# taconite/arah-release

Measured on AMD Instinct MI355X. Metric: rendered rays/sec, higher is better.
Workload: dtype f32 (operands as hi+lo f16 pairs on the f16 MFMA pipe, fp32 accumulate)

## Files before the change

arah_release_amd/csrc/arah_hip.hip:

```cpp
#include <hip/hip_runtime.h>
#include <stdint.h>
#include <stdlib.h>
#include <string.h>

#include <atomic>
#include <mutex>
#include <type_traits>

#include "../../include/arah_hip.h"
#include "pointwise.hpp"
#include "mlp.hpp"

using namespace arah;

namespace {

constexpr float kRootThresh = 1e-5f;
constexpr int kSphereIters = 50;
constexpr float kSurfaceRange = 0.05f;
constexpr float kClampDist = 0.1f;
constexpr int kBroydenSteps = 50;
constexpr float kDvg = 1.0f;
constexpr int kMaxVerts = 6912;
constexpr int kKnnThreads = 1024;
// ... 78 lines not shown
    d.vert_T = f.vert_T;
    d.bones = f.bones;
    d.scal = f.scalars;
    d.n_verts = f.n_verts;
    return d;
}

struct TierStatsRaw {
    unsigned long long rays, rays_surface, rays_promoted, rays_skipped, samples_p1, samples_p2, samples_skipped, witnesses;
    unsigned long long rays_untraced;
};
struct Counters {
    unsigned long long n_sdf_fwd, n_sdf_grad, n_skin_fwd, n_skin_jac, n_col, n_knn, n_density, n_canon, n_split_nonfinite;
    TierStatsRaw tier;
    unsigned long long n_canon_p2, n_density_p2;
    unsigned long long tier_snap[2];
    unsigned long long clk[8 * 16];
    unsigned long long clk_shade[8 * 16];
};
static_assert(offsetof(Counters, tier_snap) == sizeof(ArahCounters), "the head of Counters is the ABI's ArahCounters");
#ifdef ARAH_CLOCKS
typedef PhaseClk KernelClk;
#else
typedef NoClk KernelClk;
#endif

__device__ __forceinline__ void count_add(unsigned long long* c, int n) {
    if (c && n > 0) atomicAdd(c, (unsigned long long)n);
}

struct ColSegs {
    int n;
    int dst0[4], src0[4], len[4];
};

// ... 2401 lines not shown
        for (int s = 0; s < S; ++s)
            if (mask[base + s] != 0) step(s, z[base + s], shaded[base + s], nrm[base + s]);
    }
    step(S, 0.f, ps, pn);
    rgb[(size_t)i * 3] = any ? r : 0.f;
    rgb[(size_t)i * 3 + 1] = any ? g : 0.f;
    rgb[(size_t)i * 3 + 2] = any ? b : 0.f;
    if (acc) acc[i] = any ? fminf(fmaxf(wsum, 0.f), 1.f) : 0.f;
    vol_mask[i] = any ? 1 : 0;
    normal[(size_t)i * 3] = any ? nx : 0.f;
    normal[(size_t)i * 3 + 1] = any ? ny : 0.f;
    normal[(size_t)i * 3 + 2] = any ? nz : 0.f;
    depth[i] = any ? dz : 0.f;
}

__global__ void k_points_cam(FrameDev fr, int n, RaySet rs, const float* dists, const uint8_t* conv,
                             const float* points_hat_norm, const float* __restrict__ pose, float* points_cam) {
    const BodyConst bc = load_bc(fr);
    const int i = blockIdx.x * blockDim.x + threadIdx.x;
    if (i >= n) return;
    const V3 pw = ray_point(rs, i, dists[i]);
    const float wx = (pw.x - bc.trans[0]) + bc.trans[0], wy = (pw.y - bc.trans[1]) + bc.trans[1],
                wz = (pw.z - bc.trans[2]) + bc.trans[2];
    const float ax = fabsf(points_hat_norm[(size_t)i * 3]), ay = fabsf(points_hat_norm[(size_t)i * 3 + 1]),
                az = fabsf(points_hat_norm[(size_t)i * 3 + 2]);
    const bool surf = conv[i] && ax <= 1.0f && ay <= 1.0f && az <= 1.0f;
    for (int r = 0; r < 3; ++r) {
        const float v = pose[r * 4] * wx + pose[r * 4 + 1] * wy + pose[r * 4 + 2] * wz + pose[r * 4 + 3];
        points_cam[(size_t)i * 3 + r] = surf ? v : 0.f;
    }
// ... 38 lines not shown
    f32x4* spill;
    float *t, *far, *xcur, *Tcur, *x0raw, *grad_sdf, *jac_lbs;
    uint8_t* diverged;
    int* nn_idx;
    float *u_eval, *u_step, *u_gx, *u_Jinv, *err_best_ray, *xbest_ray, *zbest_ray;
    float *o_xnorm, *o_Tray, *o_start, *o_end, *o_acc;
    uint8_t* o_conv;
    float* q_err;
    float *o_z, *o_pts, *o_T;
    uint8_t* o_mask;
    uint8_t* q_smask;
    f32x4* shaded;
    int *listC, *listD;
    int* tcounts;
    uint8_t* ray_tier;
    size_t bytes;
};

Workspace carve(void* base, int n_rays, int n_steps) {
    Workspace w;
    Carver c{reinterpret_cast<char*>(base), 0};
    const size_t N = (size_t)(n_rays > 0 ? n_rays : 1), Q = N * (size_t)(n_steps > 0 ? n_steps : 1);
    w.ctr = c.take<Counters>(1);
    w.counts = c.take<int>(3 * kNumCounts);
    w.spill = c.take<f32x4>((size_t)kMaxGrid * kSpillPerWg);
    w.t = c.take<float>(N);
    w.far = c.take<float>(N);
    w.xcur = c.take<float>(N * 3);
    w.Tcur = c.take<float>(N * 16);
    w.x0raw = c.take<float>(N * 3);
// ... 15 lines not shown
    w.o_acc = c.take<float>(N);
    w.o_conv = c.take<uint8_t>(N);
    w.listA = c.take<int>(Q);
    w.listB = c.take<int>(Q);
    w.q_err = c.take<float>(Q);
    w.o_z = c.take<float>(Q);
    w.o_pts = c.take<float>(Q * 3);
    w.o_T = c.take<float>(Q * 16);
    w.o_mask = c.take<uint8_t>(Q);
    w.q_smask = c.take<uint8_t>(Q);
    w.shaded = c.take<f32x4>(Q);
    w.listC = c.take<int>(Q);
    w.listD = c.take<int>(Q);
    w.tcounts = c.take<int>(TC_COUNT);
    w.ray_tier = c.take<uint8_t>(N);
    w.bytes = align_up(c.off, 256);
    return w;
}

struct Knobs {
    int max_grid;
    int knn_group;
    int knn_below[3];
    int joint_bulk;
    int trace_bulk;
    int trace_small;
    bool train_b3;
    int canon_tier_wgs;
    int posed_canon;
};
// ... 812 lines not shown
    Workspace w = carve(const_cast<void*>(workspace), 1, 1);
    hipStream_t s = reinterpret_cast<hipStream_t>(stream);
    if (hipMemcpyAsync(h_out, w.ctr->clk, sizeof(w.ctr->clk) + sizeof(w.ctr->clk_shade), hipMemcpyDeviceToHost, s) != hipSuccess) return ARAH_E_LAUNCH;
    return hipStreamSynchronize(s) == hipSuccess ? ARAH_OK : ARAH_E_LAUNCH;
}
#endif

int arah_counters_read(const void* workspace, ArahCounters* h_out, void* stream) {
    if (!workspace || !h_out) return ARAH_E_BADARG;
    Workspace w = carve(const_cast<void*>(workspace), 1, 1);
    hipStream_t s = reinterpret_cast<hipStream_t>(stream);
    if (hipMemcpyAsync(h_out, w.ctr, sizeof(ArahCounters), hipMemcpyDeviceToHost, s) != hipSuccess) return ARAH_E_LAUNCH;
    return hipStreamSynchronize(s) == hipSuccess ? ARAH_OK : ARAH_E_LAUNCH;
}

int arah_sdf_eval(const ArahFrame* f, const float* x_norm, int32_t n, float* sdf, float* feat, float* grad,
                  void* workspace, size_t wbytes, void* stream) {
    if (!f || n < 0 || !workspace) return ARAH_E_BADARG;
    if (n == 0) return ARAH_OK;
    if (!x_norm || !sdf) return ARAH_E_BADARG;
    Workspace w = carve(workspace, 1, 1);
    if (wbytes < w.bytes) return ARAH_E_WORKSPACE;
    if (int arc = setup_attributes()) return arc;
    hipStream_t s = reinterpret_cast<hipStream_t>(stream);
    const FrameDev fd = to_dev(*f);
    const int g = grid_for(n, kTile);
    if (grad)
        LAUNCH_ENGINE(fd.split, (k_sdf_eval<true, true>), (k_sdf_eval<true, false>), dim3(g), dim3(kThreads), kLdsSdfGrad,
                      s, fd, x_norm, (const int*)nullptr, (const int*)nullptr, n, sdf, feat, grad, w.spill,
                      &w.ctr->n_sdf_fwd, &w.ctr->n_sdf_grad, 0);
// ... 1142 lines not shown
                         reinterpret_cast<hipStream_t>(stream));
    return check_launch();
}

static void launch_density(const FrameDev& fd, Workspace& w, const float* pts, long long Q, const int* list, const int* count,
                           int* next_list, int* next_count, hipStream_t s) {
    const int g = grid_for(Q, kTile);
    if (fd.split && Q >= 128ll * 1024)
        hipLaunchKernelGGL((k_density<true, 8>), dim3(min(num_cus(), grid_for(Q, 128))), dim3(kThreads), kLdsDensityWide, s, fd,
                           pts, list, count, w.shaded, next_list, next_count, &w.ctr->n_sdf_fwd, &w.ctr->n_density);
    else
        LAUNCH_ENGINE(fd.split, k_density<true>, k_density<false>, dim3(g), dim3(kThreads), kLdsSdfFwd, s, fd, pts, list, count,
                      w.shaded, next_list, next_count, &w.ctr->n_sdf_fwd, &w.ctr->n_density);
}

struct MapsOut {
    f32x4* nrm;
    float* normal;
    float* depth;
};

static int shade_tail(const ArahFrame* f, const ArahSampling* cfg, Workspace& w, const FrameDev& fd, const float* dirs,
                      const float* z, const float* pts, const float* T, const uint8_t* mask, int32_t n, const int* slist,
                      const int* scount, float* rgb, float* acc, uint8_t* vol_mask, const MapsOut* maps, hipStream_t s);

static int shade_impl(const ArahFrame* f, const ArahSampling* cfg, Workspace& w, const float* dirs, const float* z,
                      const float* pts, const float* T, const uint8_t* mask, int32_t n, float* rgb, float* acc,
                      uint8_t* vol_mask, const MapsOut* maps, hipStream_t s) {
    const int S = cfg->n_steps;
    const FrameDev fd = to_dev(*f);
    const long long Q = (long long)n * S;
    hipMemsetAsync(w.counts, 0, sizeof(int) * 3 * kNumCounts, s);
    hipLaunchKernelGGL(k_build_list, dim3((int)((Q + 4095) / 4096)), dim3(1024), 0, s, mask, (int)Q, w.listA, &w.counts[0]);
    const int g = grid_for(Q, kTile);
    const int* slist = w.listA;
    const int* scount = &w.counts[0];
    if (!cfg->full_shading) {
        if (cfg->ev_density[0] && cfg->ev_density[1]) hipEventRecord(reinterpret_cast<hipEvent_t>(cfg->ev_density[0]), s);
        launch_density(fd, w, pts, Q, (const int*)w.listA, (const int*)&w.counts[0], w.listB, &w.counts[1], s);
        if (cfg->ev_density[0] && cfg->ev_density[1]) hipEventRecord(reinterpret_cast<hipEvent_t>(cfg->ev_density[1]), s);
        slist = w.listB;
        scount = &w.counts[1];
    }
    return shade_tail(f, cfg, w, fd, dirs, z, pts, T, mask, n, slist, scount, rgb, acc, vol_mask, maps, s);
}

extern "C++" template <bool MAPS>
static void launch_shade(const ArahFrame* f, const ArahSampling* cfg, Workspace& w, const FrameDev& fd, const float* dirs,
                         const float* pts, const float* T, const int* slist, const int* scount, int g, f32x4* nrm,
                         hipStream_t s) {
    const int S = cfg->n_steps;
    const B3Nets b3 = b3_of(*f);
// ... 10 lines not shown
        LAUNCH_ENGINE(fd.split, (k_shade<true, true, false, MAPS>), (k_shade<true, false, false, MAPS>), dim3(g), dim3(kThreads),
                      lds_shade<true>(), s, fd, S, cfg->cano_view_dirs, dirs, pts, T, slist, scount, 0, w.shaded, w.spill,
                      &w.ctr->n_sdf_fwd, &w.ctr->n_sdf_grad, &w.ctr->n_col, b3, nrm);
    else
        LAUNCH_ENGINE(fd.split, (k_shade<false, true, false, MAPS>), (k_shade<false, false, false, MAPS>), dim3(g), dim3(kThreads),
                      lds_shade<false>(), s, fd, S, cfg->cano_view_dirs, dirs, pts, T, slist, scount, 0, w.shaded, w.spill,
                      &w.ctr->n_sdf_fwd, &w.ctr->n_sdf_grad, &w.ctr->n_col, b3, nrm);
}

static int shade_tail(const ArahFrame* f, const ArahSampling* cfg, Workspace& w, const FrameDev& fd, const float* dirs,
                      const float* z, const float* pts, const float* T, const uint8_t* mask, int32_t n, const int* slist,
                      const int* scount, float* rgb, float* acc, uint8_t* vol_mask, const MapsOut* maps, hipStream_t s) {
    const int S = cfg->n_steps;
    const long long Q = (long long)n * S;
    const int g = grid_for(Q, kTile);
    if (cfg->ev_shade[0] && cfg->ev_shade[1]) hipEventRecord(reinterpret_cast<hipEvent_t>(cfg->ev_shade[0]), s);
    if (maps) launch_shade<true>(f, cfg, w, fd, dirs, pts, T, slist, scount, g, maps->nrm, s);
    else launch_shade<false>(f, cfg, w, fd, dirs, pts, T, slist, scount, g, nullptr, s);
    if (cfg->ev_shade[0] && cfg->ev_shade[1]) hipEventRecord(reinterpret_cast<hipEvent_t>(cfg->ev_shade[1]), s);
    const bool chunk = S % 8 == 0 && (reinterpret_cast<uintptr_t>(z) & 15) == 0 && (reinterpret_cast<uintptr_t>(mask) & 7) == 0;
    const dim3 gc((n + 127) / 128), bc(128);
    if (maps) {
        if (chunk) hipLaunchKernelGGL(k_composite_maps<true>, gc, bc, 0, s, n, S, cfg->render_last_pt, z, mask, (const f32x4*)w.shaded,
                                      rgb, acc, vol_mask, (const f32x4*)maps->nrm, maps->normal, maps->depth);
        else hipLaunchKernelGGL(k_composite_maps<false>, gc, bc, 0, s, n, S, cfg->render_last_pt, z, mask, (const f32x4*)w.shaded,
                                rgb, acc, vol_mask, (const f32x4*)maps->nrm, maps->normal, maps->depth);
    } else if (chunk) hipLaunchKernelGGL(k_composite<true>, gc, bc, 0, s, n, S, cfg->render_last_pt, z, mask, (const f32x4*)w.shaded,
                                         rgb, acc, vol_mask);
    else hipLaunchKernelGGL(k_composite<false>, gc, bc, 0, s, n, S, cfg->render_last_pt, z, mask, (const f32x4*)w.shaded,
                            rgb, acc, vol_mask);
    return check_launch();
}

int arah_shade_points(const ArahFrame* f, const float* x_norm, const float* T, const float* dirs, int32_t n,
                      int32_t cano_view_dirs, int32_t shade_engine, float* rgbs, float* sdfn, void* workspace, size_t wbytes,
                      void* stream) {
// ... 1472 lines not shown
    Workspace w = carve(workspace, n, cfg->n_steps);
    if (wbytes < w.bytes) return ARAH_E_WORKSPACE;
    if (int arc = setup_attributes()) return arc;
    hipStream_t s = reinterpret_cast<hipStream_t>(stream);
    float* o_start = dists ? dists : w.o_start;
    uint8_t* o_conv = surface_conv ? surface_conv : w.o_conv;
    const uint8_t* skip = nullptr;
    if (cfg->occupancy) {
        OccBuf o = carve_occ(const_cast<void*>(cfg->occupancy));
        hipLaunchKernelGGL(k_tier_rays, dim3((n + 255) / 256), dim3(256), 0, s, n, make_rays(cam_loc, dirs, rays_per_cam), near_far,
                           (const OccInfo*)o.info, (const uint8_t*)o.dist, w.ray_tier, &w.ctr->tier);
        skip = w.ray_tier;
    }
    rc = trace_impl(f, w, cam_loc, rays_per_cam, dirs, near_far, n, 0, w.o_xnorm, w.o_Tray, o_conv, o_start, w.o_end, s, skip);
    if (rc) return rc;
    if (cfg->occupancy && !cfg->full_shading) {
        rc = render_tiers(f, cfg, w, cam_loc, rays_per_cam, dirs, near_far, o_conv, o_start, w.o_end, n, rgb,
                          acc ? acc : w.o_acc, vol_mask, maps, s);
        if (rc) return rc;
    } else {
        rc = sample_impl(f, cfg, w, cam_loc, rays_per_cam, dirs, near_far, o_conv, o_start, w.o_end, n, nullptr, nullptr,
                         nullptr, w.o_z, w.o_pts, w.o_T, w.o_mask, s);
        if (rc) return rc;
        rc = shade_impl(f, cfg, w, dirs, w.o_z, w.o_pts, w.o_T, w.o_mask, n, rgb, acc ? acc : w.o_acc, vol_mask, maps, s);
        if (rc) return rc;
    }
    if (points_cam)
        hipLaunchKernelGGL(k_points_cam, dim3((n + 255) / 256), dim3(256), 0, s, to_dev(*f), n,
                           make_rays(cam_loc, dirs, rays_per_cam), (const float*)o_start, (const uint8_t*)o_conv,
                           (const float*)w.o_xnorm, d_pose34, points_cam);
    return check_launch();
// ... 57 lines not shown
    const size_t off = align_up(c.off, 256);
    a.w = carve(base ? reinterpret_cast<char*>(base) + off : nullptr, n_rays, n_steps);
    a.bytes = off + a.w.bytes;
    return a;
}

extern "C" {
size_t arah_tier_audit_bytes(int32_t n_rays, int32_t n_steps) { return carve_audit(nullptr, n_rays, n_steps).bytes; }

int arah_tier_audit(const ArahFrame* f, const ArahSampling* cfg, const float* cam_loc, int32_t rays_per_cam, const float* dirs,
                    const float* near_far, int32_t n, int32_t rate_log2, uint32_t seed, void* audit_buf, size_t audit_bytes,
                    void* workspace, size_t wbytes, void* stream) {
    if (!f || !cfg || n < 0 || !workspace || !audit_buf) return ARAH_E_BADARG;
    int rc = check_sampling(cfg);
    if (rc) return rc;
    if (!cfg->occupancy || cfg->full_shading || rate_log2 < 0 || rate_log2 > 31) return ARAH_E_BADARG;
    if (n > 0 && (!cam_loc || !dirs || !near_far)) return ARAH_E_BADARG;
    const int S = cfg->n_steps;
    Workspace w = carve(workspace, n, S);
    if (wbytes < w.bytes) return ARAH_E_WORKSPACE;
    AuditBuf ab = carve_audit(audit_buf, n, S);
    if (audit_bytes < ab.bytes) return ARAH_E_WORKSPACE;
    if (int arc = setup_attributes()) return arc;
    hipStream_t s = reinterpret_cast<hipStream_t>(stream);
    Workspace& a = ab.w;
    hipMemsetAsync(a.ctr, 0, sizeof(Counters), s);
    hipLaunchKernelGGL(k_audit_begin, dim3(1), dim3(256), 0, s, ab.res, ab.aux, a.tcounts, (int)rate_log2, seed);
    if (n == 0) {
        hipLaunchKernelGGL(k_audit_finish, dim3(1), dim3(64), 0, s, ab.res, (const int*)ab.aux);
        return check_launch();
    }
// ... 169 lines not shown
```

arah_release_amd/hip.py:

```python
import ctypes as C
import os

import torch

_HERE = os.path.dirname(os.path.abspath(__file__))
LIB_PATH = os.environ.get("ARAH_LIB_PATH") or os.path.join(_HERE, "libarah_hip.so")

ARAH_MAX_STEPS = 128
COLOR_NO_VIEW_DIR = 0
COLOR_IDR = 1
PRECISION_SPLIT_F16 = 0
PRECISION_FP32 = 1


SHADE_ENGINE_DEFAULT, SHADE_ENGINE_FP32 = 0, 1
CANON_KERNEL_WAVE, CANON_KERNEL_TILE, CANON_KERNEL_WAVE_L2 = 0, 1, 2


def default_shade_engine():
    return SHADE_ENGINE_FP32 if os.environ.get("ARAH_SHADE_ENGINE", "b3") == "fp32" else SHADE_ENGINE_DEFAULT


def default_canon_kernel():
    return {"tile": CANON_KERNEL_TILE, "wave_l2": CANON_KERNEL_WAVE_L2}.get(os.environ.get("ARAH_CANON_KERNEL", "wave"), CANON_KERNEL_WAVE)
# ... 62 lines not shown
                ("d", _fp * 6)]


class ArahCounters(C.Structure):
    _fields_ = [("n_sdf_fwd", C.c_uint64), ("n_sdf_grad", C.c_uint64), ("n_skin_fwd", C.c_uint64),
                ("n_skin_jac", C.c_uint64), ("n_col", C.c_uint64), ("n_knn", C.c_uint64),
                ("n_density", C.c_uint64), ("n_canon", C.c_uint64), ("n_split_nonfinite", C.c_uint64),
                ("n_tier_rays", C.c_uint64), ("n_tier_rays_surface", C.c_uint64), ("n_tier_rays_promoted", C.c_uint64),
                ("n_tier_rays_skipped", C.c_uint64), ("n_tier_samples_p1", C.c_uint64), ("n_tier_samples_p2", C.c_uint64),
                ("n_tier_samples_skipped", C.c_uint64), ("n_tier_witnesses", C.c_uint64),
                ("n_tier_rays_untraced", C.c_uint64),
                ("n_canon_p2", C.c_uint64), ("n_density_p2", C.c_uint64)]


COUNTER_BYTES = C.sizeof(ArahCounters)


class ArahTierAudit(C.Structure):
    _fields_ = [("a_examined", C.c_uint64), ("a_violations", C.c_uint64), ("b_examined", C.c_uint64),
                ("b_converged", C.c_uint64), ("b_violations", C.c_uint64), ("c_examined", C.c_uint64),
                ("c_violations", C.c_uint64), ("n_first", C.c_uint64), ("first_index", C.c_int64 * 8),
                ("first_class", C.c_int32 * 8), ("min_ratio", C.c_float), ("rate_log2", C.c_int32), ("seed", C.c_uint32),
                ("reserved", C.c_int32)]


AUDIT_BYTES = C.sizeof(ArahTierAudit)

EXPORTS = ["arah_frame_bytes", "arah_prepare_frame", "arah_body_bytes", "arah_prepare_body", "arah_workspace_bytes", "arah_counters_reset",
           "arah_counters_read", "arah_sdf_eval", "arah_sdf_grid", "arah_rasterize", "arah_skin_lbs", "arah_skin_jacobian", "arah_color_eval",
           "arah_nearest_inverse_lbs", "arah_broyden3_lbs", "arah_joint_root_find", "arah_trace", "arah_sample_canonicalize",
           "arah_shade_composite", "arah_shade_points", "arah_render", "arah_shade_train_slab_bytes", "arah_shade_train_forward",
           "arah_shade_train_backward", "arah_composite_train_forward", "arah_composite_train_backward", "arah_gram_skinny_blocks", "arah_gram_skinny", "arah_colsum_blocks", "arah_colsum", "arah_inverse3x3", "arah_hsoftmax_train_forward", "arah_hsoftmax_train_backward", "arah_pose_tree_forward", "arah_pose_tree_backward", "arah_gemv_rows", "arah_mesh_query_scratch_bytes", "arah_mesh_query", "arah_dominant_kernel",
           "arah_skin_lbs_counted", "arah_marching_cubes_scratch_bytes", "arah_marching_cubes",
           "arah_marching_cubes_indexed_scratch_bytes", "arah_marching_cubes_indexed",
           "arah_occupancy_bytes", "arah_prepare_occupancy", "arah_occupancy_info", "arah_tier_debug", "arah_debug_samples",
           "arah_sample_depths_debug", "arah_cell_clusters_debug",
           "arah_sdf_grid_band_scratch_bytes", "arah_sdf_grid_band", "arah_tier_audit_bytes", "arah_tier_audit",
           "arah_tier_audit_debug", "arah_occupancy_clear_box", "arah_render_maps_bytes", "arah_render_maps",
           "arah_query_posed_bytes", "arah_query_posed", "arah_sdf_grid_posed_bytes", "arah_sdf_grid_posed",
           "arah_image_metrics_bytes", "arah_image_metrics",
           "arah_mesh_index_bytes", "arah_mesh_index_build", "arah_mesh_closest", "arah_surface_metrics_bytes", "arah_surface_metrics", "arah_face_area_cumsum",
           "arah_mesh_components_scratch_bytes", "arah_mesh_components", "arah_mesh_select_scratch_bytes", "arah_mesh_select",
           "arah_mesh_simplify_scratch_bytes", "arah_mesh_simplify",
           "arah_mesh_quadric_place_scratch_bytes", "arah_mesh_quadric_place",
# ... 235 lines not shown
            _check(load_library().arah_debug_samples(_ptr(self.buf), C.c_size_t(self.buf.numel()), C.c_int32(n_rays), C.c_int32(n_steps),
                                                     _ptr(out.get("z")), _ptr(out.get("pts")), _ptr(out.get("T")), _ptr(out.get("mask")),
                                                     _ptr(out.get("shaded")), _ptr(out.get("state")), _stream(d)), "arah_debug_samples")
        return out

    def ensure(self, n_rays, n_steps):
        need = load_library().arah_workspace_bytes(int(n_rays), int(n_steps))
        if self.buf is None or self.buf.numel() < need:
            old = self.buf
            with torch.cuda.device(self.device):
                self.buf = torch.empty(need, dtype=torch.uint8, device=self.device)
                if old is None:
                    _check(load_library().arah_counters_reset(_ptr(self.buf), _stream(self.device)),
                           "arah_counters_reset")
                else:
                    self.buf[:COUNTER_BYTES].copy_(old[:COUNTER_BYTES])
        return self.buf

    def reset_counters(self):
        with torch.cuda.device(self.device):
            _check(load_library().arah_counters_reset(_ptr(self.buf), _stream(self.device)), "arah_counters_reset")

    def counters(self):
        out = ArahCounters()
        with torch.cuda.device(self.device):
            _check(load_library().arah_counters_read(_ptr(self.buf), C.byref(out), _stream(self.device)),
                   "arah_counters_read")
        return {k: int(getattr(out, k)) for k, _ in ArahCounters._fields_}


OCC_NC, OCC_F, OCC_L, OCC_MAX_CELLS, OCC_MAX_VOX, OCC_ALIGN, TIER_BAND = 49, 3, 1.5, 12288, 1 << 22, 256, 18.0
OCC_MAX_FINE = OCC_MAX_CELLS * OCC_F ** 3
OCC_INFO_WORDS = 16
OCC_FIELDS = (("info", torch.int32, (OCC_INFO_WORDS,)), ("bits", torch.int32, (OCC_MAX_VOX // 32,)), ("dist", torch.uint8, (OCC_MAX_VOX,)),
              ("csdf", torch.float32, (OCC_NC ** 3,)), ("cpts", torch.float32, (OCC_NC ** 3, 3)),
              ("cell_lip", torch.float32, (OCC_MAX_CELLS,)), ("cell_stretch", torch.float32, (OCC_MAX_CELLS,)),
              ("fnorm", torch.float32, (OCC_MAX_FINE, 3)), ("fsdf", torch.float32, (OCC_MAX_FINE,)), ("iota", torch.int32, (OCC_MAX_FINE,)),
              ("sel_raw", torch.float32, (OCC_MAX_FINE, 3)), ("sel_bar", torch.float32, (OCC_MAX_FINE, 3)),
              ("sel_idx", torch.int32, (OCC_MAX_FINE,)), ("sel_of", torch.int32, (OCC_MAX_FINE,)))


def occupancy_layout():
    out, off = [], 0
# ... 115 lines not shown
        _same_device(*keep)
        nbytes = lib.arah_frame_bytes(C.byref(nets), C.byref(body))
        self.handle = ArahFrame()
        with _on_device(dev):
            self.buf = torch.empty(nbytes, dtype=torch.uint8, device=dev)
            _check(lib.arah_prepare_frame(C.byref(nets), C.byref(body), _ptr(self.buf), C.c_size_t(nbytes),
                                          C.byref(self.handle), _stream()), "arah_prepare_frame")
        self._keep = keep
        self.device = dev
        self.color_mode = int(color_mode)


class Sampling:

    def __init__(self, device, n_steps=64, n_near=16, n_far=16, cano_view_dirs=True, render_last_pt=False,
                 full_shading=False, shade_engine=None, canon_kernel=None):
        if n_steps < n_near + n_far + 1 or n_steps > ARAH_MAX_STEPS:
            raise ValueError("need n_near + n_far + 1 <= n_steps <= %d (ARAH_E_SAMPLING)" % ARAH_MAX_STEPS)
        self.lin_steps = torch.linspace(0.0, 1.0, n_steps, dtype=torch.float32).to(device)
        self.lin_near = torch.linspace(0.0, 1.0, n_near + 1, dtype=torch.float32).to(device)
        self.lin_far = torch.linspace(0.0, 1.0, max(n_far, 1), dtype=torch.float32).to(device)
        s = ArahSampling()
        s.n_steps, s.n_near, s.n_far = int(n_steps), int(n_near), int(n_far)
        s.cano_view_dirs, s.render_last_pt = int(bool(cano_view_dirs)), int(bool(render_last_pt))
        s.full_shading = int(bool(full_shading))
        s.lin_steps, s.lin_near, s.lin_far = _ptr(self.lin_steps), _ptr(self.lin_near), _ptr(self.lin_far)
        s.shade_engine = default_shade_engine() if shade_engine is None else int(shade_engine)
        s.canon_kernel = default_canon_kernel() if canon_kernel is None else int(canon_kernel)
        self.handle = s
        self._events = {}
        self.n_steps, self.n_near, self.n_far = n_steps, n_near, n_far

    def set_events(self, which, start=None, stop=None):
        field = getattr(self.handle, {"canon": "ev_canon", "density": "ev_density", "shade": "ev_shade", "canon2": "ev_canon2",
                                      "density2": "ev_density2"}[which])
        for ev in (start, stop):
            if ev is not None and not ev.cuda_event:
                ev.record()
        field[0] = start.cuda_event if start is not None else None
        field[1] = stop.cuda_event if stop is not None else None
# ... 1657 lines not shown
        raise ValueError("inverse3x3: (P, 3, 3) required")
    with _on_device(dev):
        out = torch.empty_like(mm)
        _check(lib.arah_inverse3x3(_ptr(mm), C.c_int32(mm.shape[0]), C.c_float(float(scale)), _ptr(out), _stream()),
               "arah_inverse3x3")
    return out


@_guarded
def render(frame, ws, sampling, cam_loc, dirs, near_far, pose34, tiered=False, maps=False):
    lib = load_library()
    cam, d, nf = _f32(cam_loc), _f32(dirs), _f32(near_far)
    n, S = d.shape[0], sampling.n_steps
    buf = ws.ensure(n, S)
    cfg = sampling.handle
    if tiered and not cfg.full_shading:
        occ = ws.occupancy(frame)
        buf = ws.buf
        cfg = ArahSampling.from_buffer_copy(sampling.handle)
        cfg.occupancy = occ.data_ptr()
    dev = d.device
    rgb = torch.empty(n, 3, device=dev)
    pcam = torch.empty(n, 3, device=dev)
    vol = torch.empty(n, dtype=torch.uint8, device=dev)
    acc = torch.empty(n, device=dev)
    dists = torch.empty(n, device=dev)
    conv = torch.empty(n, dtype=torch.uint8, device=dev)
    d_pose = _f32(pose34).reshape(-1)[:12].contiguous()
    if not maps:
        _check(lib.arah_render(C.byref(frame.handle), C.byref(cfg), _ptr(cam), C.c_int32(n // cam.shape[0]),
                               _ptr(d), _ptr(nf), _ptr(d_pose), C.c_int32(n), _ptr(rgb), _ptr(pcam), _ptr(vol), _ptr(acc),
# ... 40 lines not shown
```

arah_release_amd/renderer.py:

```python
import os

import numpy as np
import torch
import torch.nn as nn

from . import hip, training
from .nets import folded_weight


def draw_uniform(shape, device, tag):
    return torch.rand(shape, device=device)


def _emitted_sdf_layers(sdf_network):
    n = len(sdf_network)
    layers, freqs, phases = [], [], []
    for i in range(n - 1):
        lin = sdf_network[i][0]
        layers.append((lin.weights[0], lin.biases.reshape(-1)))
        freqs.append(lin.freq.reshape(-1))
        phases.append(lin.phase_shift.reshape(-1))
    last = sdf_network[n - 1]
    layers.append((last.weights[0], last.biases.reshape(-1)))
    return layers, torch.cat(freqs), torch.cat(phases)
# ... 196 lines not shown
                             "surface range, like every ARAH config")
        self.root_finding_threshold = root_finding_threshold
        self.sphere_tracing_iters = sphere_tracing_iters
        self.n_steps = n_steps
        self.near_surface_vol_samples = near_surface_vol_samples
        self.far_surface_vol_samples = far_surface_vol_samples
        self.surface_vol_range = surface_vol_range
        self.sample_bg_pts = sample_bg_pts
        self.low_vram = low_vram
        self.pending_bounds_ok = None
        self._ws = {}
        self._sampling = {}
        self.full_shading = os.environ.get("ARAH_FULL_SHADING", "0") == "1"
        self.shade_engine = None
        self.canon_kernel = None
        self._events = {}

    def workspace(self, device):
        device = torch.device(device)
        if device.type == "cuda" and device.index is None:
            device = torch.device("cuda", torch.cuda.current_device())
        key = (device, torch.cuda.current_stream(device).cuda_stream if device.type == "cuda" else 0)
        if key not in self._ws:
            if len(self._ws) >= 8:
                self._ws.pop(next(iter(self._ws)))
            self._ws[key] = hip.Workspace(device)
        return self._ws[key]

    def workspaces(self):
        return list(self._ws.values())

    def sampling(self, device, cano_view_dirs=True, render_last_pt=False, full_shading=None):
        full = bool(self.full_shading if full_shading is None else full_shading)
        key = (str(device), bool(cano_view_dirs), bool(render_last_pt), full, self.shade_engine, self.canon_kernel)
        if key not in self._sampling:
            sm = hip.Sampling(device, self.n_steps, self.near_surface_vol_samples, self.far_surface_vol_samples,
                              cano_view_dirs, render_last_pt, full, self.shade_engine, self.canon_kernel)
            for which, (a, b) in self._events.items():
                sm.set_events(which, a, b)
            self._sampling[key] = sm
        return self._sampling[key]

    def set_events(self, which, start=None, stop=None):
        if start is None or stop is None:
            self._events.pop(which, None)
        else:
            self._events[which] = (start, stop)
        for sm in self._sampling.values():
            sm.set_events(which, start, stop)

    def forward(self, sdf_network, skinning_model, cam_loc, ray_directions, body_bounds_intersections, loc,
                sc_factor, smpl_verts, smpl_verts_cano, skinning_weights, vol_feat, bone_transforms, trans,
# ... 162 lines not shown
               "surface_normals": None}
        if pred_weights is not None:
            out["pred_weights"] = pred_weights
        if inside_sdf is not None:
            out["inside_sdf"] = inside_sdf
        return out

    def _split_guard(self, ws, dev):
        key = (dev, id(ws))
        g = self._guard.get(key)
        if g is not None and self.guard_mode != "strict" and g["event"].query():
            ctr = g["host"].tolist()
            now = int(ctr[8])
            grew = now - g["seen"] if now >= g["seen"] else now
            g["seen"] = now
            d_col, d_den = ctr[4] - g["col"], ctr[6] - g["den"]
            g["col"], g["den"] = ctr[4], ctr[6]
            win_full, g["win_full"] = g["win_full"], False
            if d_den > 0 and d_col >= 0 and not win_full:
                self.shade_ratio = d_col / d_den
                self._shade_full = self.shade_ratio > 0.7
            tier_now = (ctr[13], ctr[14], ctr[15])
            d_t = [a - b for a, b in zip(tier_now, g["tier"])]
            g["tier"] = tier_now
            if min(d_t) >= 0 and sum(d_t) > 0:
                self.tier_share = d_t[2] / sum(d_t)
                self._tier_off = self.tier_share < 1.0 / 3.0
            if grew > 0:
                self.split_nonfinite += grew
                if self._precision != hip.PRECISION_FP32:
                    import warnings
                    warnings.warn("split-f16 engine: %d loop-C samples met activations outside the f16 range; following frames "
                                  "use the exact fp32 engine (ARAH_PRECISION=fp32)" % grew)
                    self._precision = hip.PRECISION_FP32
        if g is None:
            if len(self._guard) >= 8:
                self._guard.pop(next(iter(self._guard)))
            g = self._guard[key] = {"host": torch.zeros(hip.COUNTER_BYTES // 8, dtype=torch.int64).pin_memory(), "event": torch.cuda.Event(),
                                    "seen": 0, "col": 0, "den": 0, "win_full": False, "tier": (0, 0, 0)}
        return g

    def _split_guard_arm(self, g, ws, full=False):
        g["win_full"] = g["win_full"] or bool(full)
        g["host"].copy_(ws.buf[0:hip.COUNTER_BYTES].view(torch.int64), non_blocking=True)
        g["event"].record()

    def _tier_audit_mode(self):
        mode = self.tier_audit
        if mode not in ("off", "sample", "strict"):
            raise ValueError("tier_audit must be 'off', 'sample' or 'strict', not %r" % (mode,))
        return mode

    def _tier_audit_violated(self, res, where):
        import warnings
        self.tier_violations += res["violations"]
        self.tier_audit_last = res
        self.tiering = False
        warnings.warn("tiered forward: the audit of the sigma = +0 certificate found %d violation(s) (classes A/B/C: %d/%d/%d, "
                      "min sdf / beta %.3g); %s, and the following frames render untiered until `tiering` is set again"
# ... 653 lines not shown
```

include/arah_hip.h:

```cpp
#ifndef ARAH_HIP_H
#define ARAH_HIP_H

#include <stddef.h>
#include <stdint.h>

#ifdef __cplusplus
extern "C" {
#endif

#define ARAH_OK 0
#define ARAH_E_BADARG (-1)
#define ARAH_E_SHAPE (-2)
#define ARAH_E_WORKSPACE (-3)
#define ARAH_E_LAUNCH (-4)
#define ARAH_E_SAMPLING (-5)
#define ARAH_E_OVERFLOW (-6)

#define ARAH_MAX_STEPS 128
#define ARAH_N_JOINTS 24
#define ARAH_COLOR_NO_VIEW_DIR 0
#define ARAH_COLOR_IDR 1

#define ARAH_PRECISION_SPLIT_F16 0
#define ARAH_PRECISION_FP32 1
// ... 14 lines not shown
    int32_t precision;
} ArahNets;

typedef struct ArahBody {
    const float* verts;
    const float* vert_weights;
    const float* bones;
    const float* trans;
    const float* center;
    const float* coord_min;
    const float* coord_max;
    int32_t n_verts;
    const void* prepared;
} ArahBody;

enum { ARAH_SHADE_ENGINE_DEFAULT = 0 , ARAH_SHADE_ENGINE_FP32 = 1 };
enum { ARAH_CANON_KERNEL_WAVE = 0 , ARAH_CANON_KERNEL_TILE = 1,
       ARAH_CANON_KERNEL_WAVE_L2 = 2 };

typedef struct ArahSampling {
    int32_t n_steps, n_near, n_far;
    int32_t cano_view_dirs;
    int32_t render_last_pt;
    int32_t full_shading;
    const float* lin_steps;
    const float* lin_near;
    const float* lin_far;
    int32_t shade_engine;
    int32_t canon_kernel;
    void* ev_canon[2];
// ... 61 lines not shown
    uint64_t n_tier_rays, n_tier_rays_surface, n_tier_rays_promoted, n_tier_rays_skipped;
    uint64_t n_tier_samples_p1, n_tier_samples_p2, n_tier_samples_skipped, n_tier_witnesses;
    uint64_t n_tier_rays_untraced;
    uint64_t n_canon_p2, n_density_p2;
} ArahCounters;

size_t arah_body_bytes(void);
int arah_prepare_body(const float* verts, int32_t n_verts, void* body_buf, size_t body_bytes, void* stream);
size_t arah_frame_bytes(const ArahNets* h_nets, const ArahBody* h_body);
int arah_prepare_frame(const ArahNets* h_nets, const ArahBody* h_body, void* frame_buf, size_t frame_bytes,
                       ArahFrame* h_frame_out, void* stream);

size_t arah_workspace_bytes(int32_t n_rays, int32_t n_steps);
int arah_counters_reset(void* workspace, void* stream);
int arah_counters_read(const void* workspace, ArahCounters* h_out, void* stream);

int arah_sdf_eval(const ArahFrame* h_frame, const float* x_norm, int32_t n_pts, float* sdf, float* feat,
                  float* grad, void* workspace, size_t workspace_bytes, void* stream);
int arah_sdf_grid(const ArahFrame* h_frame, int32_t n_side, float* sdf, void* workspace, size_t workspace_bytes,
                  void* stream);
size_t arah_sdf_grid_band_scratch_bytes(void);
int arah_sdf_grid_band(const ArahFrame* h_frame, int32_t n_side, float* sdf, int32_t* list, void* scratch,
                       size_t scratch_bytes, void* workspace, size_t workspace_bytes, void* stream);
int arah_rasterize(const float* tri_uvz, int32_t n_faces, int32_t height, int32_t width, float z_near,
                   uint64_t* zbuf, void* stream);
int arah_skin_lbs(const ArahFrame* h_frame, const float* x_hat, int32_t n_pts, float* w, float* x_bar,
                  float* T, void* workspace, size_t workspace_bytes, void* stream);
int arah_skin_lbs_counted(const ArahFrame* h_frame, const float* x_hat, int32_t n_max, const int32_t* n_items,
                          int32_t per_item, float* x_bar, void* workspace, size_t workspace_bytes, void* stream);
size_t arah_marching_cubes_scratch_bytes(int32_t n_side);
// ... 292 lines not shown
```

Measured before the change: 11.60 million.

## Cull color shading for samples with negligible transmittance-weighted contribution, with rescue pass

Adds a lazy shading path that first runs a density-only compositing pass to tag samples whose weight cannot change the accumulated sum, then runs the color MLP only on the remaining head samples. The composite then checks whether the culled samples could have changed rgb and, for rays where they could, shades the culled samples in a rescue pass and composites those rays again. This cuts color network evaluations for samples late in the ray. In exchange it adds extra split and composite kernels, a memset and a second shade launch, and it needs more workspace and counter plumbing.

```diff
diff --git a/arah_release_amd/csrc/arah_hip.hip b/arah_release_amd/csrc/arah_hip.hip
--- a/arah_release_amd/csrc/arah_hip.hip
+++ b/arah_release_amd/csrc/arah_hip.hip
@@ -116,11 +116,12 @@
     unsigned long long n_sdf_fwd, n_sdf_grad, n_skin_fwd, n_skin_jac, n_col, n_knn, n_density, n_canon, n_split_nonfinite;
     TierStatsRaw tier;
     unsigned long long n_canon_p2, n_density_p2;
+    unsigned long long n_shade_culled, n_shade_rescued;
     unsigned long long tier_snap[2];
     unsigned long long clk[8 * 16];
     unsigned long long clk_shade[8 * 16];
 };
-static_assert(offsetof(Counters, tier_snap) == sizeof(ArahCounters), "the head of Counters is the ABI's ArahCounters");
+static_assert(offsetof(Counters, n_shade_culled) == sizeof(ArahCounters), "the head of Counters is the ABI's ArahCounters");
 #ifdef ARAH_CLOCKS
 typedef PhaseClk KernelClk;
 #else
@@ -2552,6 +2553,179 @@
     depth[i] = any ? dz : 0.f;
 }
 
+__global__ void k_cull_mark(const int* __restrict__ list, const int* __restrict__ count, int S, uint8_t* __restrict__ ray_pos) {
+    const int n = *count;
+    for (int i = blockIdx.x * blockDim.x + threadIdx.x; i < n; i += gridDim.x * blockDim.x) ray_pos[list[i] / S] = 1;
+}
+
+__device__ __forceinline__ void append_sample_bits(unsigned long long m0, unsigned long long m1, int base, int* list, int* count) {
+    const int lane = threadIdx.x & 63;
+    const int cnt = __popcll(m0) + __popcll(m1);
+    int incl = cnt;
+#pragma unroll
+    for (int d = 1; d < 64; d <<= 1) {
+        const int t = __shfl_up(incl, d);
+        if (lane >= d) incl += t;
+    }
+    const int total = __shfl(incl, 63);
+    int o = 0;
+    if (lane == 63 && total) o = atomicAdd(count, total);
+    o = __shfl(o, 63) + incl - cnt;
+    for (; m0; m0 &= m0 - 1) list[o++] = base + __ffsll((long long)m0) - 1;
+    for (; m1; m1 &= m1 - 1) list[o++] = base + 64 + __ffsll((long long)m1) - 1;
+}
+
+__device__ __forceinline__ void wave_count_add(unsigned long long* ctr, int v) {
+#pragma unroll
+    for (int d = 32; d > 0; d >>= 1) v += __shfl_xor(v, d);
+    if ((threadIdx.x & 63) == 0) count_add(ctr, v);
+}
+
+template <bool CHUNK>
+__global__ __launch_bounds__(128) void k_shade_split(int n, int S, int render_last_pt, const float* __restrict__ z,
+                                                     const uint8_t* __restrict__ mask, const f32x4* __restrict__ shaded,
+                                                     const uint8_t* __restrict__ ray_pos, uint8_t* __restrict__ tag,
+                                                     int* __restrict__ head, int* head_count) {
+#pragma clang fp contract(off)
+    const int i = blockIdx.x * blockDim.x + threadIdx.x;
+    unsigned long long h0 = 0ull, h1 = 0ull;
+    const size_t base = (size_t)(i < n ? i : 0) * S;
+    if (i < n && ray_pos[i]) {
+        const float inv_steps = 1.0f / (float)S;
+        float ws = 0.f, trans = 1.0f, pd = 0.f, pz = 0.f;
+        int prev = -1;
+        auto step = [&](int s, float zs, float dens) {
+            if (prev >= 0) {
+                float delta;
+                if (s < S) delta = zs - pz;
+                else delta = render_last_pt ? 1e10f : inv_steps;
+                const float alpha = 1.0f - expf(-pd * delta);
+                const float w = alpha * trans;
+                if (pd > 0.f) {
+                    const bool tail = ws + 8.0f * w == ws;
+                    tag[base + prev] = tail ? 1 : 0;
+                    if (!tail) {
+                        if (prev < 64) h0 |= 1ull << prev;
+                        else h1 |= 1ull << (prev - 64);
+                    }
+                }
+                ws = fmaf(alpha, trans, ws);
+                trans *= (1.0f - alpha + 1e-7f);
+            }
+            if (s < S) {
+                prev = s;
+                pd = dens;
+                pz = zs;
+            }
+        };
+        if (CHUNK) {
+            typedef unsigned u32x2 __attribute__((ext_vector_type(2)));
+            for (int s0 = 0; s0 < S; s0 += 8) {
+                const u32x2 m8 = *reinterpret_cast<const u32x2*>(mask + base + s0);
+                const f32x4 z0 = *reinterpret_cast<const f32x4*>(z + base + s0), z1 = *reinterpret_cast<const f32x4*>(z + base + s0 + 4);
+                float d8[8];
+#pragma unroll
+                for (int u = 0; u < 8; ++u) d8[u] = shaded[base + s0 + u][3];
+#pragma unroll
+                for (int u = 0; u < 8; ++u)
+                    if (((u < 4 ? m8[0] : m8[1]) >> (8 * (u & 3))) & 0xffu) step(s0 + u, u < 4 ? z0[u & 3] : z1[u & 3], d8[u]);
+            }
+        } else {
+            for (int s = 0; s < S; ++s)
+                if (mask[base + s] != 0) step(s, z[base + s], shaded[base + s][3]);
+        }
+        step(S, 0.f, 0.f);
+    }
+    append_sample_bits(h0, h1, (int)base, head, head_count);
+}
+
+template <bool CHUNK, bool RESCUE>
+__global__ __launch_bounds__(128) void k_composite_cull(int n, int S, int render_last_pt, const float* __restrict__ z,
+                                                        const uint8_t* __restrict__ mask, const f32x4* __restrict__ shaded,
+                                                        const uint8_t* __restrict__ tag, uint8_t* ray_flag, int* __restrict__ rescue,
+                                                        int* rescue_count, float* __restrict__ rgb, float* __restrict__ acc,
+                                                        uint8_t* __restrict__ vol_mask, unsigned long long* ctr_culled,
+                                                        unsigned long long* ctr_rescued) {
+#pragma clang fp contract(off)
+    const int i = blockIdx.x * blockDim.x + threadIdx.x;
+    const bool live = i < n && (!RESCUE || ray_flag[i] != 0);
+    if (RESCUE && !live) return;
+    const size_t base = (size_t)(i < n ? i : 0) * S;
+    unsigned long long t0 = 0ull, t1 = 0ull;
+    bool bad = false;
+    if (live) {
+        const float inv_steps = 1.0f / (float)S;
+        float r = 0.f, g = 0.f, b = 0.f, wsum = 0.f, trans = 1.0f;
+        int prev = -1;
+        f32x4 ps = {0.f, 0.f, 0.f, 0.f};
+        float pz = 0.f;
+        bool any = false, ptail = false;
+        auto step = [&](int s, float zs, const f32x4 sh, bool tail) {
+            if (prev >= 0) {
+                float delta;
+                if (s < S) delta = zs - pz;
+                else delta = render_last_pt ? 1e10f : inv_steps;
+                const float alpha = 1.0f - expf(-ps[3] * delta);
+                const float w = alpha * trans;
+                if (!RESCUE && ptail) {
+                    const float w2 = 2.0f * w;
+                    bad = bad || !(r + w2 == r && g + w2 == g && b + w2 == b);
+                    if (prev < 64) t0 |= 1ull << prev;
+                    else t1 |= 1ull << (prev - 64);
+                }
+                r = fmaf(ps[0], w, r);
+                g = fmaf(ps[1], w, g);
+                b = fmaf(ps[2], w, b);
+                wsum = fmaf(alpha, trans, wsum);
+                trans *= (1.0f - alpha + 1e-7f);
+            }
+            if (s < S) {
+                prev = s;
+                ps = sh;
+                pz = zs;
+                ptail = tail;
+                any = true;
+            }
+        };
+        if (CHUNK) {
+            typedef unsigned u32x2 __attribute__((ext_vector_type(2)));
+            for (int s0 = 0; s0 < S; s0 += 8) {
+                const u32x2 m8 = *reinterpret_cast<const u32x2*>(mask + base + s0);
+                const f32x4 z0 = *reinterpret_cast<const f32x4*>(z + base + s0), z1 = *reinterpret_cast<const f32x4*>(z + base + s0 + 4);
+                u32x2 t8 = {0u, 0u};
+                if (!RESCUE) t8 = *reinterpret_cast<const u32x2*>(tag + base + s0);
+                f32x4 sh[8];
+#pragma unroll
+                for (int u = 0; u < 8; ++u) sh[u] = shaded[base + s0 + u];
+#pragma unroll
+                for (int u = 0; u < 8; ++u)
+                    if (((u < 4 ? m8[0] : m8[1]) >> (8 * (u & 3))) & 0xffu)
+                        step(s0 + u, u < 4 ? z0[u & 3] : z1[u & 3], sh[u],
+                             !RESCUE && sh[u][3] > 0.f && (((u < 4 ? t8[0] : t8[1]) >> (8 * (u & 3))) & 0xffu) != 0u);
+            }
+        } else {
+            for (int s = 0; s < S; ++s)
+                if (mask[base + s] != 0) {
+                    const f32x4 sh = shaded[base + s];
+                    step(s, z[base + s], sh, !RESCUE && sh[3] > 0.f && tag[base + s] != 0);
+                }
+        }
+        step(S, 0.f, ps, false);
+        rgb[(size_t)i * 3] = any ? r : 0.f;
+        rgb[(size_t)i * 3 + 1] = any ? g : 0.f;
+        rgb[(size_t)i * 3 + 2] = any ? b : 0.f;
+        if (acc) acc[i] = any ? fminf(fmaxf(wsum, 0.f), 1.f) : 0.f;
+        vol_mask[i] = any ? 1 : 0;
+        if (!RESCUE) ray_flag[i] = bad ? 1 : 0;
+    }
+    if (!RESCUE) {
+        const int n_tail = __popcll(t0) + __popcll(t1);
+        wave_count_add(ctr_culled, bad ? 0 : n_tail);
+        wave_count_add(ctr_rescued, bad ? n_tail : 0);
+        append_sample_bits(bad ? t0 : 0ull, bad ? t1 : 0ull, (int)base, rescue, rescue_count);
+    }
+}
+
 __global__ void k_points_cam(FrameDev fr, int n, RaySet rs, const float* dists, const uint8_t* conv,
                              const float* points_hat_norm, const float* __restrict__ pose, float* points_cam) {
     const BodyConst bc = load_bc(fr);
@@ -2620,6 +2794,8 @@
     int *listC, *listD;
     int* tcounts;
     uint8_t* ray_tier;
+    uint8_t* cull_tag;
+    uint8_t* cull_ray;
     size_t bytes;
 };
 
@@ -2665,6 +2841,8 @@
     w.listD = c.take<int>(Q);
     w.tcounts = c.take<int>(TC_COUNT);
     w.ray_tier = c.take<uint8_t>(N);
+    w.cull_tag = c.take<uint8_t>(Q);
+    w.cull_ray = c.take<uint8_t>(256 + N);
     w.bytes = align_up(c.off, 256);
     return w;
 }
@@ -3507,6 +3685,14 @@
     return hipStreamSynchronize(s) == hipSuccess ? ARAH_OK : ARAH_E_LAUNCH;
 }
 
+int arah_shade_cull_counters(const void* workspace, uint64_t* h_out2, void* stream) {
+    if (!workspace || !h_out2) return ARAH_E_BADARG;
+    Workspace w = carve(const_cast<void*>(workspace), 1, 1);
+    hipStream_t s = reinterpret_cast<hipStream_t>(stream);
+    if (hipMemcpyAsync(h_out2, &w.ctr->n_shade_culled, 2 * sizeof(uint64_t), hipMemcpyDeviceToHost, s) != hipSuccess) return ARAH_E_LAUNCH;
+    return hipStreamSynchronize(s) == hipSuccess ? ARAH_OK : ARAH_E_LAUNCH;
+}
+
 int arah_sdf_eval(const ArahFrame* f, const float* x_norm, int32_t n, float* sdf, float* feat, float* grad,
                   void* workspace, size_t wbytes, void* stream) {
     if (!f || n < 0 || !workspace) return ARAH_E_BADARG;
@@ -4679,6 +4865,10 @@
                       w.shaded, next_list, next_count, &w.ctr->n_sdf_fwd, &w.ctr->n_density);
 }
 
+static bool shade_everything(const ArahSampling* cfg) {
+    return cfg->full_shading != ARAH_SHADING_LAZY && cfg->full_shading != ARAH_SHADING_LAZY_NO_CULL;
+}
+
 struct MapsOut {
     f32x4* nrm;
     float* normal;
@@ -4700,7 +4890,7 @@
     const int g = grid_for(Q, kTile);
     const int* slist = w.listA;
     const int* scount = &w.counts[0];
-    if (!cfg->full_shading) {
+    if (!shade_everything(cfg)) {
         if (cfg->ev_density[0] && cfg->ev_density[1]) hipEventRecord(reinterpret_cast<hipEvent_t>(cfg->ev_density[0]), s);
         launch_density(fd, w, pts, Q, (const int*)w.listA, (const int*)&w.counts[0], w.listB, &w.counts[1], s);
         if (cfg->ev_density[0] && cfg->ev_density[1]) hipEventRecord(reinterpret_cast<hipEvent_t>(cfg->ev_density[1]), s);
@@ -4741,12 +4931,41 @@
     const int S = cfg->n_steps;
     const long long Q = (long long)n * S;
     const int g = grid_for(Q, kTile);
+    const bool chunk = S % 8 == 0 && (reinterpret_cast<uintptr_t>(z) & 15) == 0 && (reinterpret_cast<uintptr_t>(mask) & 7) == 0;
+    const dim3 gc((n + 127) / 128), bc(128);
+    if (cfg->full_shading == ARAH_SHADING_LAZY && !maps) {
+        int* ccount = reinterpret_cast<int*>(w.cull_ray);
+        uint8_t* ray_flag = w.cull_ray + 256;
+        int *head = w.listC, *rescue = w.listD;
+        const f32x4* shaded = w.shaded;
+        hipMemsetAsync(w.cull_ray, 0, 256 + (size_t)n, s);
+        hipLaunchKernelGGL(k_cull_mark, dim3(min(1024, grid_for(Q, 256))), dim3(256), 0, s, slist, scount, S, ray_flag);
+        if (chunk) hipLaunchKernelGGL(k_shade_split<true>, gc, bc, 0, s, n, S, cfg->render_last_pt, z, mask, shaded,
+                                      (const uint8_t*)ray_flag, w.cull_tag, head, &ccount[0]);
+        else hipLaunchKernelGGL(k_shade_split<false>, gc, bc, 0, s, n, S, cfg->render_last_pt, z, mask, shaded,
+                                (const uint8_t*)ray_flag, w.cull_tag, head, &ccount[0]);
+        if (cfg->ev_shade[0] && cfg->ev_shade[1]) hipEventRecord(reinterpret_cast<hipEvent_t>(cfg->ev_shade[0]), s);
+        launch_shade<false>(f, cfg, w, fd, dirs, pts, T, head, &ccount[0], g, nullptr, s);
+        if (cfg->ev_shade[0] && cfg->ev_shade[1]) hipEventRecord(reinterpret_cast<hipEvent_t>(cfg->ev_shade[1]), s);
+        if (chunk) hipLaunchKernelGGL((k_composite_cull<true, false>), gc, bc, 0, s, n, S, cfg->render_last_pt, z, mask, shaded,
+                                      (const uint8_t*)w.cull_tag, ray_flag, rescue, &ccount[1], rgb, acc, vol_mask,
+                                      &w.ctr->n_shade_culled, &w.ctr->n_shade_rescued);
+        else hipLaunchKernelGGL((k_composite_cull<false, false>), gc, bc, 0, s, n, S, cfg->render_last_pt, z, mask, shaded,
+                                (const uint8_t*)w.cull_tag, ray_flag, rescue, &ccount[1], rgb, acc, vol_mask,
+                                &w.ctr->n_shade_culled, &w.ctr->n_shade_rescued);
+        launch_shade<false>(f, cfg, w, fd, dirs, pts, T, rescue, &ccount[1], g, nullptr, s);
+        if (chunk) hipLaunchKernelGGL((k_composite_cull<true, true>), gc, bc, 0, s, n, S, cfg->render_last_pt, z, mask, shaded,
+                                      (const uint8_t*)nullptr, ray_flag, (int*)nullptr, (int*)nullptr, rgb, acc, vol_mask,
+                                      (unsigned long long*)nullptr, (unsigned long long*)nullptr);
+        else hipLaunchKernelGGL((k_composite_cull<false, true>), gc, bc, 0, s, n, S, cfg->render_last_pt, z, mask, shaded,
+                                (const uint8_t*)nullptr, ray_flag, (int*)nullptr, (int*)nullptr, rgb, acc, vol_mask,
+                                (unsigned long long*)nullptr, (unsigned long long*)nullptr);
+        return check_launch();
+    }
     if (cfg->ev_shade[0] && cfg->ev_shade[1]) hipEventRecord(reinterpret_cast<hipEvent_t>(cfg->ev_shade[0]), s);
     if (maps) launch_shade<true>(f, cfg, w, fd, dirs, pts, T, slist, scount, g, maps->nrm, s);
     else launch_shade<false>(f, cfg, w, fd, dirs, pts, T, slist, scount, g, nullptr, s);
     if (cfg->ev_shade[0] && cfg->ev_shade[1]) hipEventRecord(reinterpret_cast<hipEvent_t>(cfg->ev_shade[1]), s);
-    const bool chunk = S % 8 == 0 && (reinterpret_cast<uintptr_t>(z) & 15) == 0 && (reinterpret_cast<uintptr_t>(mask) & 7) == 0;
-    const dim3 gc((n + 127) / 128), bc(128);
     if (maps) {
         if (chunk) hipLaunchKernelGGL(k_composite_maps<true>, gc, bc, 0, s, n, S, cfg->render_last_pt, z, mask, (const f32x4*)w.shaded,
                                       rgb, acc, vol_mask, (const f32x4*)maps->nrm, maps->normal, maps->depth);
@@ -6249,7 +6468,7 @@
     }
     rc = trace_impl(f, w, cam_loc, rays_per_cam, dirs, near_far, n, 0, w.o_xnorm, w.o_Tray, o_conv, o_start, w.o_end, s, skip);
     if (rc) return rc;
-    if (cfg->occupancy && !cfg->full_shading) {
+    if (cfg->occupancy && !shade_everything(cfg)) {
         rc = render_tiers(f, cfg, w, cam_loc, rays_per_cam, dirs, near_far, o_conv, o_start, w.o_end, n, rgb,
                           acc ? acc : w.o_acc, vol_mask, maps, s);
         if (rc) return rc;
@@ -6337,7 +6556,7 @@
     if (!f || !cfg || n < 0 || !workspace || !audit_buf) return ARAH_E_BADARG;
     int rc = check_sampling(cfg);
     if (rc) return rc;
-    if (!cfg->occupancy || cfg->full_shading || rate_log2 < 0 || rate_log2 > 31) return ARAH_E_BADARG;
+    if (!cfg->occupancy || shade_everything(cfg) || rate_log2 < 0 || rate_log2 > 31) return ARAH_E_BADARG;
     if (n > 0 && (!cam_loc || !dirs || !near_far)) return ARAH_E_BADARG;
     const int S = cfg->n_steps;
     Workspace w = carve(workspace, n, S);
diff --git a/arah_release_amd/hip.py b/arah_release_amd/hip.py
--- a/arah_release_amd/hip.py
+++ b/arah_release_amd/hip.py
@@ -100,6 +100,8 @@
 
 
 COUNTER_BYTES = C.sizeof(ArahCounters)
+CULL_COUNTER_BYTES = 16
+SHADING_LAZY, SHADING_FULL, SHADING_LAZY_NO_CULL = 0, 1, 2
 
 
 class ArahTierAudit(C.Structure):
@@ -113,7 +115,7 @@
 AUDIT_BYTES = C.sizeof(ArahTierAudit)
 
 EXPORTS = ["arah_frame_bytes", "arah_prepare_frame", "arah_body_bytes", "arah_prepare_body", "arah_workspace_bytes", "arah_counters_reset",
-           "arah_counters_read", "arah_sdf_eval", "arah_sdf_grid", "arah_rasterize", "arah_skin_lbs", "arah_skin_jacobian", "arah_color_eval",
+           "arah_counters_read", "arah_shade_cull_counters", "arah_sdf_eval", "arah_sdf_grid", "arah_rasterize", "arah_skin_lbs", "arah_skin_jacobian", "arah_color_eval",
            "arah_nearest_inverse_lbs", "arah_broyden3_lbs", "arah_joint_root_find", "arah_trace", "arah_sample_canonicalize",
            "arah_shade_composite", "arah_shade_points", "arah_render", "arah_shade_train_slab_bytes", "arah_shade_train_forward",
            "arah_shade_train_backward", "arah_composite_train_forward", "arah_composite_train_backward", "arah_gram_skinny_blocks", "arah_gram_skinny", "arah_colsum_blocks", "arah_colsum", "arah_inverse3x3", "arah_hsoftmax_train_forward", "arah_hsoftmax_train_backward", "arah_pose_tree_forward", "arah_pose_tree_backward", "arah_gemv_rows", "arah_mesh_query_scratch_bytes", "arah_mesh_query", "arah_dominant_kernel",
@@ -379,7 +381,7 @@
                     _check(load_library().arah_counters_reset(_ptr(self.buf), _stream(self.device)),
                            "arah_counters_reset")
                 else:
-                    self.buf[:COUNTER_BYTES].copy_(old[:COUNTER_BYTES])
+                    self.buf[:COUNTER_BYTES + CULL_COUNTER_BYTES].copy_(old[:COUNTER_BYTES + CULL_COUNTER_BYTES])
         return self.buf
 
     def reset_counters(self):
@@ -391,7 +393,12 @@
         with torch.cuda.device(self.device):
             _check(load_library().arah_counters_read(_ptr(self.buf), C.byref(out), _stream(self.device)),
                    "arah_counters_read")
-        return {k: int(getattr(out, k)) for k, _ in ArahCounters._fields_}
+            cull = (C.c_uint64 * 2)()
+            _check(load_library().arah_shade_cull_counters(_ptr(self.buf), cull, _stream(self.device)),
+                   "arah_shade_cull_counters")
+        res = {k: int(getattr(out, k)) for k, _ in ArahCounters._fields_}
+        res["n_shade_culled"], res["n_shade_rescued"] = int(cull[0]), int(cull[1])
+        return res
 
 
 OCC_NC, OCC_F, OCC_L, OCC_MAX_CELLS, OCC_MAX_VOX, OCC_ALIGN, TIER_BAND = 49, 3, 1.5, 12288, 1 << 22, 256, 18.0
@@ -537,7 +544,7 @@
 class Sampling:
 
     def __init__(self, device, n_steps=64, n_near=16, n_far=16, cano_view_dirs=True, render_last_pt=False,
-                 full_shading=False, shade_engine=None, canon_kernel=None):
+                 full_shading=False, shade_engine=None, canon_kernel=None, shade_cull=True):
         if n_steps < n_near + n_far + 1 or n_steps > ARAH_MAX_STEPS:
             raise ValueError("need n_near + n_far + 1 <= n_steps <= %d (ARAH_E_SAMPLING)" % ARAH_MAX_STEPS)
         self.lin_steps = torch.linspace(0.0, 1.0, n_steps, dtype=torch.float32).to(device)
@@ -546,7 +553,7 @@
         s = ArahSampling()
         s.n_steps, s.n_near, s.n_far = int(n_steps), int(n_near), int(n_far)
         s.cano_view_dirs, s.render_last_pt = int(bool(cano_view_dirs)), int(bool(render_last_pt))
-        s.full_shading = int(bool(full_shading))
+        s.full_shading = SHADING_FULL if full_shading else (SHADING_LAZY if shade_cull else SHADING_LAZY_NO_CULL)
         s.lin_steps, s.lin_near, s.lin_far = _ptr(self.lin_steps), _ptr(self.lin_near), _ptr(self.lin_far)
         s.shade_engine = default_shade_engine() if shade_engine is None else int(shade_engine)
         s.canon_kernel = default_canon_kernel() if canon_kernel is None else int(canon_kernel)
@@ -2234,7 +2241,7 @@
     n, S = d.shape[0], sampling.n_steps
     buf = ws.ensure(n, S)
     cfg = sampling.handle
-    if tiered and not cfg.full_shading:
+    if tiered and cfg.full_shading != SHADING_FULL:
         occ = ws.occupancy(frame)
         buf = ws.buf
         cfg = ArahSampling.from_buffer_copy(sampling.handle)
diff --git a/arah_release_amd/renderer.py b/arah_release_amd/renderer.py
--- a/arah_release_amd/renderer.py
+++ b/arah_release_amd/renderer.py
@@ -234,6 +234,7 @@
         self.full_shading = os.environ.get("ARAH_FULL_SHADING", "0") == "1"
         self.shade_engine = None
         self.canon_kernel = None
+        self.shade_cull = True
         self._events = {}
 
     def workspace(self, device):
@@ -252,10 +253,11 @@
 
     def sampling(self, device, cano_view_dirs=True, render_last_pt=False, full_shading=None):
         full = bool(self.full_shading if full_shading is None else full_shading)
-        key = (str(device), bool(cano_view_dirs), bool(render_last_pt), full, self.shade_engine, self.canon_kernel)
+        key = (str(device), bool(cano_view_dirs), bool(render_last_pt), full, self.shade_engine, self.canon_kernel,
+               bool(self.shade_cull))
         if key not in self._sampling:
             sm = hip.Sampling(device, self.n_steps, self.near_surface_vol_samples, self.far_surface_vol_samples,
-                              cano_view_dirs, render_last_pt, full, self.shade_engine, self.canon_kernel)
+                              cano_view_dirs, render_last_pt, full, self.shade_engine, self.canon_kernel, self.shade_cull)
             for which, (a, b) in self._events.items():
                 sm.set_events(which, a, b)
             self._sampling[key] = sm
@@ -448,8 +450,9 @@
             now = int(ctr[8])
             grew = now - g["seen"] if now >= g["seen"] else now
             g["seen"] = now
-            d_col, d_den = ctr[4] - g["col"], ctr[6] - g["den"]
-            g["col"], g["den"] = ctr[4], ctr[6]
+            col = ctr[4] + ctr[20]
+            d_col, d_den = col - g["col"], ctr[6] - g["den"]
+            g["col"], g["den"] = col, ctr[6]
             win_full, g["win_full"] = g["win_full"], False
             if d_den > 0 and d_col >= 0 and not win_full:
                 self.shade_ratio = d_col / d_den
@@ -470,13 +473,13 @@
         if g is None:
             if len(self._guard) >= 8:
                 self._guard.pop(next(iter(self._guard)))
-            g = self._guard[key] = {"host": torch.zeros(hip.COUNTER_BYTES // 8, dtype=torch.int64).pin_memory(), "event": torch.cuda.Event(),
+            g = self._guard[key] = {"host": torch.zeros((hip.COUNTER_BYTES + hip.CULL_COUNTER_BYTES) // 8, dtype=torch.int64).pin_memory(), "event": torch.cuda.Event(),
                                     "seen": 0, "col": 0, "den": 0, "win_full": False, "tier": (0, 0, 0)}
         return g
 
     def _split_guard_arm(self, g, ws, full=False):
         g["win_full"] = g["win_full"] or bool(full)
-        g["host"].copy_(ws.buf[0:hip.COUNTER_BYTES].view(torch.int64), non_blocking=True)
+        g["host"].copy_(ws.buf[0:hip.COUNTER_BYTES + hip.CULL_COUNTER_BYTES].view(torch.int64), non_blocking=True)
         g["event"].record()
 
     def _tier_audit_mode(self):
diff --git a/include/arah_hip.h b/include/arah_hip.h
--- a/include/arah_hip.h
+++ b/include/arah_hip.h
@@ -52,6 +52,7 @@
     const void* prepared;
 } ArahBody;
 
+enum { ARAH_SHADING_LAZY = 0, ARAH_SHADING_FULL = 1, ARAH_SHADING_LAZY_NO_CULL = 2 };
 enum { ARAH_SHADE_ENGINE_DEFAULT = 0 , ARAH_SHADE_ENGINE_FP32 = 1 };
 enum { ARAH_CANON_KERNEL_WAVE = 0 , ARAH_CANON_KERNEL_TILE = 1,
        ARAH_CANON_KERNEL_WAVE_L2 = 2 };
@@ -143,6 +144,7 @@
 size_t arah_workspace_bytes(int32_t n_rays, int32_t n_steps);
 int arah_counters_reset(void* workspace, void* stream);
 int arah_counters_read(const void* workspace, ArahCounters* h_out, void* stream);
+int arah_shade_cull_counters(const void* workspace, uint64_t* h_out2, void* stream);
 
 int arah_sdf_eval(const ArahFrame* h_frame, const float* x_norm, int32_t n_pts, float* sdf, float* feat,
                   float* grad, void* workspace, size_t workspace_bytes, void* stream);
```

After: 12.39 million, median of 6. 1.07x the previous value.
